# lastz/lastz

Hardware: AMD Instinct MI355X
Metric: Gbp-of-target aligned/sec (whole job, --nogapped HSP path, both strands) (higher is better)
Workload: dtype s32

## Files before the change

lastz_amd/csrc/lz_common.hpp:

```cpp
#pragma once
#include <stdint.h>

#if defined(__HIP__)
#define LZ_HD __host__ __device__ inline __attribute__((always_inline))
#else
#define LZ_HD inline
#endif

typedef uint8_t  u8;
typedef uint32_t u32;
typedef int32_t  s32;
typedef uint64_t u64;
typedef int64_t  s64;

#define LZ_MAX_PARTS   16
#define LZ_MAX_PROBES  128
#define LZ_FILL_GROUP  16
#define LZ_DIAG_BITS   16
#define LZ_DIAG_SIZE   (1u << LZ_DIAG_BITS)
#define LZ_NCLASS      32
#define LZ_SEQ_PAD     64

#define LZ_CODE_CLASS(c)   ((c) & 31u)
#define LZ_CODE_BITS(c)    (((c) >> 5) & 3u)
#define LZ_CODE_INVALID    0x80u

struct LzSeedDev {
    s32 length, weight, nparts;
    s32 shift[LZ_MAX_PARTS];
    u32 mask[LZ_MAX_PARTS];
    s32 nprobes;
    u32 probe_xor[LZ_MAX_PROBES];
};

struct LzHspRec {
    u32 seed_pos1, seed_pos2;
    u32 end1;
    u32 length;
    s32 score;
};

LZ_HD u32 lz_apply_seed(const LzSeedDev& sd, u64 w)
{
    u32 packed = 0;
    for (int p = 0; p < sd.nparts; p++) packed |= (u32)(w >> sd.shift[p]) & sd.mask[p];
    return packed;
}

LZ_HD bool lz_window_word(const u8* code, u32 pos, const LzSeedDev& sd, u32& packed)
{
    u64 w = 0; u32 bad = 0;
    const u8* p = code + pos - (u32)sd.length;
    for (int k = 0; k < sd.length; k++) { u32 c = p[k]; bad |= c; w = (w << 2) | LZ_CODE_BITS(c); }
    if (bad & LZ_CODE_INVALID) return false;
    packed = lz_apply_seed(sd, w);
    return true;
}

LZ_HD u32 lz_count_hits_at(const u8* qcode, u32 pos2, u32 lo, const LzSeedDev& sd, const u32* wstart, bool& valid, u32& packed)
{
    valid = false;
    if (pos2 < lo + (u32)sd.length) return 0;
    if (!lz_window_word(qcode, pos2, sd, packed)) return 0;
    valid = true;
    u32 n = 0;
    for (int p = 0; p < sd.nprobes; p++) { u32 w = packed ^ sd.probe_xor[p]; n += wstart[w + 1] - wstart[w]; }
    return n;
}

LZ_HD u64 lz_hit_key(u32 pos1, u32 pos2) { return ((u64)(u32)(pos1 - pos2) << 32) | (u64)pos2; }

LZ_HD void lz_fill_hits_at(const u8* qcode, u32 pos2, const LzSeedDev& sd, const u32* wstart, const u32* wpos, u64* out)
{
    u32 packed;
    if (!lz_window_word(qcode, pos2, sd, packed)) return;
    for (int p = 0; p < sd.nprobes; p++) {
        u32 w = packed ^ sd.probe_xor[p];
        u32 a = wstart[w], b = wstart[w + 1];
        for (u32 j = a; j < b; j++) *out++ = lz_hit_key(wpos[j], pos2);
    }
}

#define LZ_SELF_OFF       0
#define LZ_SELF_SAME      1
#define LZ_SELF_OPP       2
#define LZ_SELF_OPP_PARTS 3
#define LZ_SELF_WINDOW    4
struct LzSelfDev {
    u32 mode, L, len2, band;
    const u32* sep1; u32 n_sep1;
    u32 wlo;
    const u32* sep2; u32 n_sep2;
// ... 461 lines not shown
```

lastz_amd/csrc/settle_kernels.hip:

```cpp
#include <hip/hip_runtime.h>
#include <cstdio>
#include "lz_ctx.hpp"
#include "lz_lut.hpp"
#include "lz_tile_runs.hpp"
#include "lz_coop.hpp"
#include "lz_seed_dev.hpp"

#define LZ_PP_TPB    1024
#define LZ_PP_WAVES  (LZ_PP_TPB / 64)
#define LZ_PP_ROUNDS (LZ_PP_TILE_HOST / LZ_PP_TPB)
#define LZ_PP_TILE   (LZ_PP_TPB * LZ_PP_ROUNDS)
#define LZ_NBIN      256
static_assert(LZ_PP_TILE == LZ_PP_TILE_HOST, "lz_tile_runs.hpp addresses runs by the tile size");

__device__ __forceinline__ u32 lz_exscan256(u32 v, u32* wtot )
{
    const u32 tid = threadIdx.x, lane = tid & 63u, w = tid >> 6;
    u32 inc = v;
#pragma unroll
    for (int d = 1; d < 64; d <<= 1) { const u32 t = __shfl_up(inc, d); if ((int)lane >= d) inc += t; }
    if (tid < 256 && lane == 63) wtot[w] = inc;
    __syncthreads();
    u32 pre = 0;
    if (tid < 256) for (u32 k = 0; k < w; k++) pre += wtot[k];
// ... 139 lines not shown
                tv = lz_load16(P.tcode + t0); qv = lz_load16(P.qcode + (t0 - diag));
            }
#pragma unroll
            for (int j = 0; j < LZ_COOP_BLK; j++) {
                const u32 tb = right ? LZ_VBYTE(tv, j) : LZ_VBYTE(tv, LZ_COOP_BLK - 1 - j);
                const u32 qb = right ? LZ_VBYTE(qv, j) : LZ_VBYTE(qv, LZ_COOP_BLK - 1 - j);
                sc[j] = tab[(LZ_CODE_CLASS(tb) << 5) | LZ_CODE_CLASS(qb)];
            }
        }
        LzCoopMap f; s32 mx; u32 jmx;
        lz_coop_block(sc, nb, X, f, mx, jmx);
        LzCoopMap inc = f;
#pragma unroll
        for (int d = 1; d < 32; d <<= 1) { const LzCoopMap g = lz_coop_shfl_up32(inc, d); if ((int)hl >= d) inc = lz_coop_compose(g, inc); }
        LzCoopMap ex = lz_coop_shfl_up32(inc, 1);
        if (hl == 0) ex = lz_coop_identity(X);
        const s32 m0 = run0 - best0 + X;
        const bool dead_before = lz_coop_fails(ex, m0);
        const s32 mi = lz_coop_apply(ex, m0), ri = run0 + ex.C;
        const bool fails_here = nb && !dead_before && lz_coop_fails(f, mi);
        const u64 fboth = __ballot(fails_here);
        const u32 fmask = right ? (u32)(fboth >> 32) : (u32)fboth;
        long long key = -1;
        u32 used_here = 0;
        if (fails_here) {
            u32 used; bool stopped; s32 rmx; u32 rj;
            lz_coop_resolve(sc, nb, X, mi, ri, used, stopped, rmx, rj);
            used_here = used;
            if (rj) key = (((long long)rmx + LZ_COOP_INF) << 16) | (long long)(0xFFFFu - (off + rj));
        } else if (nb && jmx && !dead_before)
            key = (((long long)ri + mx + LZ_COOP_INF) << 16) | (long long)(0xFFFFu - (off + jmx));
#pragma unroll
        for (int d = 16; d > 0; d >>= 1) { const long long o = __shfl_xor(key, d, 32); if (o > key) key = o; }
        const int fl = fmask ? (int)__ffs((int)fmask) - 1 : 0;
        const u32 used_f = (u32)__shfl((int)used_here, fl, 32);
        const s32 totc = __shfl(inc.C, 31, 32);
        if (alive) {
            u32 used_total;
            if (fmask) { used_total = LZ_COOP_BLK * (u32)fl + used_f; alive = false; }
            else {
                used_total = room < (u32)(LZ_COOP_BLK * LZ_COOP_LANES) ? room : (u32)(LZ_COOP_BLK * LZ_COOP_LANES);
                if (room <= (u32)(LZ_COOP_BLK * LZ_COOP_LANES)) alive = false;
            }
            if (key >= 0) {
                const s32 v = (s32)((key >> 16) - LZ_COOP_INF); const u32 idx = 0xFFFFu - (u32)(key & 0xFFFF);
                if (v > best0) { best0 = v; out.best_pos = right ? s + idx : s - idx; }
            }
            run0 += totc;
            s = right ? s + used_total : s - used_total;
        }
    }
    out.stop_pos = s; out.best = best0;
    return out;
}

#if defined(LZ_PHASE_CLOCKS)
__device__ unsigned long long g_phase_clk[6];
void lz_phase_clocks_print()
{
    unsigned long long h[6];
    if (hipMemcpyFromSymbol(h, HIP_SYMBOL(g_phase_clk), sizeof(h)) != hipSuccess) return;
    fprintf(stderr, "[lzgpu phase clocks] settle (walker work, walker barrier wait, sorter work, sorter barrier wait, extensions of wave 0: cycles, count; cycles summed over the 256 partitions):");
    for (int k = 0; k < 6; k++) fprintf(stderr, " %llu", h[k]);
    fprintf(stderr, "\n");
}
#define LZ_S2_CLK_BEGIN(who) unsigned long long _s2a = (who) ? __builtin_readcyclecounter() : 0ull, _s2b = 0ull
#define LZ_S2_CLK_MID(who, slot) do { if (who) { _s2b = __builtin_readcyclecounter(); atomicAdd(&g_phase_clk[slot], _s2b - _s2a); } } while (0)
#define LZ_S2_CLK_END(who, slot) do { if (who) atomicAdd(&g_phase_clk[slot], __builtin_readcyclecounter() - _s2b); } while (0)
#define LZ_S2_CLK_EXT_BEGIN(who, m) const unsigned long long _s2x = (who) ? __builtin_readcyclecounter() : 0ull; const unsigned _s2n = (unsigned)__popcll(m)
#define LZ_S2_CLK_EXT_END(who) do { if (who) { atomicAdd(&g_phase_clk[4], __builtin_readcyclecounter() - _s2x); atomicAdd(&g_phase_clk[5], (unsigned long long)_s2n); } } while (0)
#else
#define LZ_S2_CLK_BEGIN(who)
#define LZ_S2_CLK_MID(who, slot)
#define LZ_S2_CLK_END(who, slot)
#define LZ_S2_CLK_EXT_BEGIN(who, m)
#define LZ_S2_CLK_EXT_END(who)
void lz_phase_clocks_print() {}
#endif

#define LZ_S2_TPB     1024
#define LZ_ST_BATCH   4
#define LZ_S2_WALKW   4
#define LZ_S2_SORTW   (LZ_S2_TPB / 64 - LZ_S2_WALKW)
#define LZ_S2_ROUNDS  7
#define LZ_S2_TILE    (LZ_S2_SORTW * 64 * LZ_S2_ROUNDS)
struct LzSettle2Shared {
    s32 tab[LZ_NCLASS * LZ_NCLASS];
    u64 rec[2][LZ_S2_TILE + LZ_ST_BATCH];
    u64 bm[LZ_S2_SORTW][LZ_NBIN];
    u32 cnt[2][LZ_S2_SORTW][LZ_NBIN];
    u32 woff[LZ_S2_SORTW][LZ_NBIN];
    u32 lbeg[2][LZ_NBIN], lcnt[2][LZ_NBIN];
    alignas(8) u8 own[LZ_S2_SORTW][64 * LZ_S2_ROUNDS];
};
static_assert(sizeof(LzSettle2Shared) <= 160 * 1024, "k_settle2: one workgroup per CU");
static_assert(LZ_TR_BLOCK <= 255 && (64 * LZ_S2_ROUNDS) % 8 == 0, "own[] holds 1 + a block entry per byte, cleared 8 at a time");
__global__ void __launch_bounds__(LZ_S2_TPB)
k_settle2(LzExtendParams P, const u64* __restrict__ recs, u32 n_pp_tiles, const u32* __restrict__ hist, const u32* __restrict__ hist_part,
          const u32* __restrict__ run_addr, const u32* __restrict__ bin_base, u32* __restrict__ diag_end,
          const s32* __restrict__ score_tab_g, LzHspRec* __restrict__ out, u32* __restrict__ out_count, u32 out_cap,
          u64* __restrict__ counters)
{
    extern __shared__ __align__(16) unsigned char lz_s2_smem[];
    LzSettle2Shared& sh = *reinterpret_cast<LzSettle2Shared*>(lz_s2_smem);
    const u32 tid = threadIdx.x, lane = tid & 63u;
    const u32 w = (u32)__builtin_amdgcn_readfirstlane((int)(tid >> 6));
    const u32 part = blockIdx.x;
    const u32 r0 = bin_base[part], r1 = bin_base[part + 1];
    const u32 n = r1 - r0, ntiles = (n + LZ_S2_TILE - 1) / LZ_S2_TILE;
    if (ntiles == 0) return;
    for (u32 k = tid; k < LZ_NCLASS * LZ_NCLASS; k += LZ_S2_TPB) sh.tab[k] = score_tab_g[k];
    for (u32 k = tid; k < LZ_S2_SORTW * LZ_NBIN; k += LZ_S2_TPB) (&sh.bm[0][0])[k] = 0ull;
    const bool walker = w < LZ_S2_WALKW;
    const u32 sw = w - LZ_S2_WALKW;

    u64 cx[LZ_S2_ROUNDS], nx[LZ_S2_ROUNDS];
    u32 cslot[LZ_S2_ROUNDS];
    u32 cur = 0, bf[LZ_TR_K], ba[LZ_TR_K];
    auto load_block = [&]() {
#pragma unroll
        for (int j = 0; j < LZ_TR_K; j++) {
            const u32 t = cur + lane * LZ_TR_K + (u32)j;
            bf[j] = lz_tr_first(hist, hist_part, n_pp_tiles, t, part, r1);
            ba[j] = t < n_pp_tiles ? run_addr[(size_t)t * LZ_NBIN + part] : 0u;
        }
    };
    auto block_end = [&]() -> u32 { return (u32)__builtin_amdgcn_readlane((int)bf[LZ_TR_K - 1], 63); };
    auto window_first = [&](u32 tt) -> u32 { return r0 + tt * (u32)LZ_S2_TILE + sw * (64u * LZ_S2_ROUNDS); };
    auto advance_early = [&](u32 tt) {
        if (tt < ntiles && window_first(tt) < r1 && lz_tr_block_behind(block_end(), window_first(tt))) { cur += LZ_TR_BLOCK - 1; load_block(); }
    };
    auto load_tile = [&](u32 tt, u64* x) {
#pragma unroll
        for (int rr = 0; rr < LZ_S2_ROUNDS; rr++) x[rr] = ~0ull;
        const u32 g0 = window_first(tt);
        if (tt >= ntiles || g0 >= r1) return;
        const u32 g1 = (r1 - g0 < 64u * LZ_S2_ROUNDS) ? r1 : g0 + 64u * LZ_S2_ROUNDS;
        u8* const own = sh.own[sw];
        u32 idx[LZ_S2_ROUNDS] = {};
        for (;;) {
            const u32 bend = block_end();
            if (!lz_tr_block_behind(bend, g0)) {
                if (lane < 64u * LZ_S2_ROUNDS / 8u) reinterpret_cast<u64*>(own)[lane] = 0ull;
                u32 dl[LZ_TR_K];
#pragma unroll
                for (int j = 0; j < LZ_TR_K; j++) {
                    const u32 nf = j + 1 < LZ_TR_K ? bf[(j + 1) % LZ_TR_K] : (u32)__shfl_down((int)bf[0], 1);
                    u32 pos;
                    const bool m = lz_tr_mark(bf[j], nf, g0, g1, pos) && !(j == LZ_TR_K - 1 && lane == 63u);
                    if (m) own[pos] = (u8)(1u + lane * LZ_TR_K + (u32)j);
                    dl[j] = lz_tr_delta(ba[j], bf[j]);
                }
                const u32 bfirst = (u32)__builtin_amdgcn_readlane((int)bf[0], 0);
                u32 carry = 0;
#pragma unroll
                for (int rr = 0; rr < LZ_S2_ROUNDS; rr++) {
                    const u32 g = g0 + (u32)rr * 64u + lane;
                    const u32 mk = own[(u32)rr * 64u + lane];
                    u32 v = mk;
                    LZ_WAVE_SCAN_U32(v, mk, lz_umax)
                    v = lz_umax(v, carry);
                    carry = (u32)__builtin_amdgcn_readlane((int)v, 63);
                    const u32 e = v - 1u;
                    u32 d = (u32)__shfl((int)dl[0], (int)(e / LZ_TR_K));
#pragma unroll
                    for (int j = 1; j < LZ_TR_K; j++) { const u32 dj = (u32)__shfl((int)dl[j], (int)(e / LZ_TR_K)); if (e % LZ_TR_K == (u32)j) d = dj; }
                    if (lz_tr_covers(g, bfirst, bend, g1)) idx[rr] = lz_tr_index(g, d);
                }
                if (bend >= g1) break;
            }
            cur += LZ_TR_BLOCK - 1; load_block();
        }
#pragma unroll
        for (int rr = 0; rr < LZ_S2_ROUNDS; rr++)
            if (g0 + (u32)rr * 64u + lane < g1) x[rr] = LZ_NT_LD(recs + (size_t)idx[rr]);
    };
    auto count_tile = [&](u32 tt, const u64* x, u32* slot) {
        u32* const row = sh.cnt[tt & 1u][sw];
        reinterpret_cast<uint4*>(row)[lane] = make_uint4(0u, 0u, 0u, 0u);
        u64* const bmr = sh.bm[sw];
#pragma unroll
        for (int rr = 0; rr < LZ_S2_ROUNDS; rr++) {
            const bool valid = x[rr] != ~0ull;
            const u32 b = LZ_REC_LOW8(x[rr]);
            if (valid) atomicOr((unsigned long long*)&bmr[b], 1ull << lane);
            const u64 peers = valid ? bmr[b] : 0ull;
            const u32 old = valid ? row[b] : 0u;
            const u32 rank = (u32)__popcll(peers & ((1ull << lane) - 1ull));
            if (valid && (peers >> lane) == 1ull) { row[b] = old + (u32)__popcll(peers); bmr[b] = 0ull; }
            slot[rr] = old + rank;
        }
    };
    auto place_tile = [&](u32 tt, const u64* x, const u32* slot) {
        const u32 (*cn)[LZ_NBIN] = sh.cnt[tt & 1u];
        uint4 tot = make_uint4(0u, 0u, 0u, 0u), pre = tot;
#pragma unroll
        for (u32 k = 0; k < LZ_S2_SORTW; k++) {
            const uint4 v = reinterpret_cast<const uint4*>(cn[k])[lane];
            if (k == sw) pre = tot;
            tot.x += v.x; tot.y += v.y; tot.z += v.z; tot.w += v.w;
        }
        const u32 mine = tot.x + tot.y + tot.z + tot.w;
        u32 inc = mine;
#pragma unroll
        for (int d = 1; d < 64; d <<= 1) { const u32 t = __shfl_up(inc, d); if ((int)lane >= d) inc += t; }
        const u32 b0 = inc - mine, b1 = b0 + tot.x, b2 = b1 + tot.y, b3 = b2 + tot.z;
        reinterpret_cast<uint4*>(sh.woff[sw])[lane] = make_uint4(b0 + pre.x, b1 + pre.y, b2 + pre.z, b3 + pre.w);
        if (sw == 0) {
            reinterpret_cast<uint4*>(sh.lbeg[tt & 1u])[lane] = make_uint4(b0, b1, b2, b3);
            reinterpret_cast<uint4*>(sh.lcnt[tt & 1u])[lane] = tot;
        }
        u64* const dst = sh.rec[tt & 1u];
#pragma unroll
        for (int rr = 0; rr < LZ_S2_ROUNDS; rr++)
            if (x[rr] != ~0ull) dst[sh.woff[sw][LZ_REC_LOW8(x[rr])] + slot[rr]] = x[rr];
    };

    __syncthreads();
    if (!walker) {
        load_block();
        load_tile(0, cx); load_tile(1, nx); count_tile(0, cx, cslot);
        __syncthreads();
        place_tile(0, cx, cslot);
#pragma unroll
        for (int rr = 0; rr < LZ_S2_ROUNDS; rr++) cx[rr] = nx[rr];
        load_tile(2, nx);
        count_tile(1, cx, cslot);
        __syncthreads();
        for (u32 t = 0; t < ntiles; t++) {
            LZ_S2_CLK_BEGIN(sw == 0 && lane == 0);
            advance_early(t + 3);
            if (t + 1 < ntiles) place_tile(t + 1, cx, cslot);
#pragma unroll
            for (int rr = 0; rr < LZ_S2_ROUNDS; rr++) cx[rr] = nx[rr];
            load_tile(t + 3, nx);
            if (t + 2 < ntiles) count_tile(t + 2, cx, cslot);
            LZ_S2_CLK_MID(sw == 0 && lane == 0, 2);
            __syncthreads();
            LZ_S2_CLK_END(sw == 0 && lane == 0, 3);
        }
        return;
    }
    __syncthreads();
    __syncthreads();
    constexpr u32 BPW = LZ_NBIN / LZ_S2_WALKW;
    const bool wl = lane < BPW;
    const u32 bucket = (w * BPW + lane) & (LZ_NBIN - 1);
    const u32 h = part * LZ_NBIN + bucket;
    const u32 L = P.seed_len;
    u32 dend = wl ? diag_end[h] : 0u;
    u64 n_ext = 0, n_bp = 0;
    for (u32 t = 0; t < ntiles; t++) {
        LZ_S2_CLK_BEGIN(tid == 0);
        {
            const u64* const rec = sh.rec[t & 1u];
            u32 p = wl ? sh.lbeg[t & 1u][bucket] : 0u; const u32 end = wl ? p + sh.lcnt[t & 1u][bucket] : 0u;
            u32 ne = 0, nb = 0;
            for (;;) {
                bool pending = false; u32 pp2 = 0, ppay = 0;
                while (__ballot(p < end && !pending)) {
                    u64 r[LZ_ST_BATCH];
#pragma unroll
                    for (int k = 0; k < LZ_ST_BATCH; k++) r[k] = rec[p + k];
                    bool live = !pending;
                    u32 np = 0;
#pragma unroll
                    for (int k = 0; k < LZ_ST_BATCH; k++) {
                        const u32 p2 = LZ_REC_POS2(r[k]), pay = LZ_REC_PAYLOAD(r[k]);
                        const bool in = live && (p + (u32)k < end);
                        const bool drop = dend > p2 - L;
                        const bool slow = LZ_REC_SLOW(r[k]) != 0 && !drop;
                        const bool go = in && !slow;
                        const bool fast = go && !drop;
                        const u32 room = p2 - dend, dlo = pay & 0xFFu, dext = pay >> 8;
                        const u32 extent = p2 + dext;
                        ne += fast ? 1u : 0u;
                        nb += fast ? (dlo < room ? dlo : room) + dext : 0u;
                        dend = (fast && extent > dend) ? extent : dend;
                        np += go ? 1u : 0u;
                        if (in && slow) { pending = true; pp2 = p2; ppay = pay; }
                        live = go;
                    }
                    p += np;
                }
                u64 mask = __ballot(pending);
                if (!mask) break;
                LZ_S2_CLK_EXT_BEGIN(tid == 0, mask);
                while (mask) {
                    const int src = (int)__ffsll((long long)mask) - 1;
                    mask &= mask - 1;
                    const u32 sp2 = (u32)__shfl((int)pp2, src), spay = (u32)__shfl((int)ppay, src), sdend = (u32)__shfl((int)dend, src);
                    const u32 sh_ = part * LZ_NBIN + w * BPW + (u32)src;
                    const s32 diag = (s32)((spay << 16) | sh_);
// ... 89 lines not shown
```

lastz_amd/csrc/lz_lut.hpp:

```cpp
#pragma once
#include "lz_common.hpp"

#define LZ_PAD2         128
#define LZ_LUT_ENTRIES  4096
#define LZ_LUT_TOTAL    (2 * LZ_LUT_ENTRIES)
#define LZ_LUT_WIN_G    15
#define LZ_LUT_WIN_B    60
#define LZ_LUT_MAXWIN   3
#define LZ_GRAY(c)      ((c) ^ ((c) >> 1))

struct alignas(8) LzLutEntry { u32 ab; u32 sc; };

struct LzLutParams {
    const u8* t2; const u8* q2;
    const u8* tsp; const u8* qsp;
    const u8* t2x; const u8* tspx;
    const u8* tcode; const u8* qcode;
    s32 xdrop;
};

struct LzLutScan { u32 s; s32 run, best; u32 room, used, alive, nwin; };

#if defined(__HIP_DEVICE_COMPILE__)
LZ_HD u32 lz_alignbit(u32 hi, u32 lo, u32 sh) { return __builtin_amdgcn_alignbit(hi, lo, sh); }
// ... 123 lines not shown
            stop = stop | (on && nr < best - X);
        }
    } else if (r) {
        const s32 p1 = lz_sdot4m(sc, 0x00000001u, m), p2 = lz_sdot4m(sc, 0x00000101u, m), p3 = lz_sdot4m(sc, 0x00010101u, m), p4 = lz_sdot4(sc, m);
        const s32 q2 = p1 | p2, q3 = q2 | p3;
        j = 4u + (u32)(p1 >> 31) + (u32)(q2 >> 31) + (u32)(q3 >> 31);
        stop = (q3 | p4) < 0;
    }
    st.run = run; st.best = best;
    st.used += 4u * np + j;
    st.nwin++;
    if (stop) st.alive = 0;
    else if (r == 4u) st.alive = 2;
    else if (soft) {
        if constexpr (SPECIAL) {
            const u32 p1 = RIGHT ? st.s + lim : st.s - 1u - lim;
            const s32 v = ctab[(LZ_CODE_CLASS(P.tcode[(s64)p1]) << 5) | LZ_CODE_CLASS(P.qcode[(s64)p1 - (s64)diag])];
            st.run += v; st.used += 1u;
            if (st.run > st.best) st.best = st.run;
            const u32 eaten = lim + 1u;
            if (st.run < st.best - X || eaten == st.room) st.alive = 0;
            else { st.alive = 1; st.room -= eaten; st.s = RIGHT ? st.s + eaten : st.s - eaten; }
        }
    }
    else if (lim == st.room) st.alive = 0;
    else { st.alive = 1; st.room -= (u32)LZ_LUT_WIN_B; st.s = RIGHT ? st.s + (u32)LZ_LUT_WIN_B : st.s - (u32)LZ_LUT_WIN_B; }
}
template <bool SPECIAL, bool LIMCHK>
LZ_HD void lz_lut_window_pair(const LzLutParams& P, const LzLutEntry* lut, s32 diag, LzLutScan& L, LzLutScan& R,
                              const LzLutRaw<SPECIAL>& rawl, const LzLutRaw<SPECIAL>& rawr, bool do_l, bool do_r, const s32* ctab = nullptr)
{
    if (do_l) lz_lut_window<false, SPECIAL, LIMCHK>(P, lut, diag, L, rawl, ctab);
    if (do_r) lz_lut_window<true, SPECIAL, LIMCHK>(P, lut, diag, R, rawr, ctab);
}
template <bool RIGHT, bool SPECIAL>
LZ_HD void lz_lut_step(const LzLutParams& P, const LzLutEntry* lut, s32 diag, LzLutScan& st, const s32* ctab = nullptr)
{
    LzLutRaw<SPECIAL> raw;
    lz_lut_fetch<RIGHT, SPECIAL>(P, st.s, diag, raw);
    if (!SPECIAL && st.room >= (u32)LZ_LUT_WIN_B) lz_lut_window<RIGHT, SPECIAL, false>(P, lut, diag, st, raw);
    else                                           lz_lut_window<RIGHT, SPECIAL, true>(P, lut, diag, st, raw, ctab);
}

LZ_HD void lz_lut_init(u64 key, u32 tlen, u32 qlen, s32& diag, LzLutScan& L, LzLutScan& R)
{
    const u32 pos2 = (u32)key;
    diag = (s32)(u32)(key >> 32);
    const u32 pos1 = pos2 + (u32)diag;
    const s32 stopl = diag > 0 ? diag : 0;
    const s32 stopr = ((s32)tlen <= (s32)qlen + diag) ? (s32)tlen : (s32)qlen + diag;
    L.s = R.s = pos1; L.run = L.best = R.run = R.best = 0; L.used = R.used = 0; L.nwin = R.nwin = 0;
    L.room = (u32)((s32)pos1 - stopl); R.room = (u32)(stopr - (s32)pos1);
    L.alive = ((s32)pos1 > stopl) ? 1u : 0u; R.alive = ((s32)pos1 < stopr) ? 1u : 0u;
}

LZ_HD u32 lz_lut_summary(const LzLutScan& L, const LzLutScan& R, s32 min_score)
{
    u32 summ = (L.used & 0xFFu) | ((R.used & 0xFFu) << 8);
    if (L.alive || R.alive || L.best + R.best >= min_score) summ |= LZ_SUMM_SLOW;
    return summ;
}

template <bool SPECIAL>
LZ_HD u32 lz_lut_probe_hit(const LzLutParams& P, const LzLutEntry* lut, u32 tlen, u32 qlen, s32 min_score, u64 key, const s32* ctab = nullptr)
{
    s32 diag; LzLutScan L, R;
    lz_lut_init(key, tlen, qlen, diag, L, R);
    while (L.alive == 1 && L.nwin < (u32)LZ_LUT_MAXWIN) lz_lut_step<false, SPECIAL>(P, lut, diag, L, ctab);
    while (R.alive == 1 && R.nwin < (u32)LZ_LUT_MAXWIN) lz_lut_step<true, SPECIAL>(P, lut, diag, R, ctab);
    return lz_lut_summary(L, R, min_score);
}

LZ_HD u64 lz_hit_record(u64 key, u32 summ)
{
    const u32 pos2 = (u32)key, diag = (u32)(key >> 32);
    const bool slow = (summ & LZ_SUMM_SLOW) != 0;
    const u64 payload = slow ? (u64)(diag >> 16) : (u64)(summ & 0xFFFFu);
    return (u64)pos2 | ((u64)(diag & 0xFFu) << 31) | (payload << 39) | (slow ? (1ull << 63) : 0ull);
}
#define LZ_REC_TAG(r)     ((u32)((r) >> 55) & 0xFFu)
#define LZ_REC_UNTAG(r)   ((r) & ~(0xFFull << 55))
LZ_HD u64 lz_hit_record_tagged(u64 key, u32 summ) { return lz_hit_record(key, summ) | ((u64)((u32)(key >> 40) & 0xFFu) << 55); }

#define LZ_WCTX_BYTES 32
struct alignas(16) LzWctx { u32 w[LZ_WCTX_BYTES / 4]; };
LZ_HD u32 lz_wctx_first_byte(u32 pos1) { return ((pos1 - 1u + (u32)LZ_PAD2) >> 2) - 15u; }
LZ_HD u32 lz_wctx_right_offset(u32 pos1) { return ((pos1 + (u32)LZ_PAD2) >> 2) - lz_wctx_first_byte(pos1); }
LZ_HD LzWctx lz_wctx_make(const u8* two, u32 pos1) { LzWctx e; __builtin_memcpy(&e, two + lz_wctx_first_byte(pos1), LZ_WCTX_BYTES); return e; }
LZ_HD void lz_wctx_windows(const LzWctx& e, u32 pos1, LzVec16& tl, LzVec16& tr)
{
    const bool at16 = lz_wctx_right_offset(pos1) == 16u;
    LZ_UNROLL_ALL
    for (int k = 0; k < 4; k++) {
        tl.w[k] = e.w[k];
        const u32 at15 = lz_alignbit(e.w[4 + k], e.w[3 + k], 24u);
        tr.w[k] = at16 ? e.w[4 + k] : at15;
    }
}

#define LZ_REC_POS2(r)    ((u32)((r) & 0x7FFFFFFFu))
#define LZ_REC_LOW8(r)    ((u32)((r) >> 31) & 0xFFu)
#define LZ_REC_PAYLOAD(r) ((u32)((r) >> 39) & 0xFFFFu)
#define LZ_REC_SLOW(r)    ((u32)((r) >> 63))
LZ_HD u64 lz_rec_with_index(u64 r, u32 idx)
{ return (r & ~((0xFFull << 31) | (0x1Full << 55))) | ((u64)(idx & 0xFFu) << 31) | ((u64)((idx >> 8) & 0x1Fu) << 55); }
#define LZ_REC_INDEX(r)   (((u32)((r) >> 31) & 0xFFu) | (((u32)((r) >> 55) & 0x1Fu) << 8))

template <class Emit>
LZ_HD void lz_settle_record(const LzExtendParams& P, const s32* score_tab, u64 rec, u32 h ,
                            u32& dend, u64& n_ext, u64& n_bp, Emit&& emit)
{
    const u32 p2 = LZ_REC_POS2(rec);
    if (dend > p2 - P.seed_len) return;
    n_ext++;
    const u32 pay = LZ_REC_PAYLOAD(rec);
    if (!LZ_REC_SLOW(rec)) {
        const u32 room = p2 - dend, dlo = pay & 0xFFu, dext = pay >> 8;
        const u32 extent = p2 + dext;
        n_bp += (dlo < room ? dlo : room) + dext;
        if (extent > dend) dend = extent;
        return;
    }
    const s32 diag = (s32)((pay << 16) | h);
    dend = lz_reextend(P, score_tab, p2, diag, dend, n_bp, emit);
}
```

lastz_amd/csrc/scan_kernels.hip:

```cpp
#include <hip/hip_runtime.h>
#include <algorithm>
#include <type_traits>
#include "lz_ctx.hpp"
#include "lz_host.hpp"
#include "lz_lut.hpp"
#include "lz_seed_dev.hpp"

#define LZ_SC_ROUNDS 4

struct LzScanTask { u32 idx; s32 diag; LzLutScan L, R; };
static_assert(sizeof(LzScanTask) == 64, "LzScanTask: one 64-byte line per task");
#define LZ_SC_TPB 512
template <int MODE> struct LzScanShared {
    union {
        LzLutEntry lut[LZ_LUT_TOTAL];
        struct { s32 tab[LZ_NCLASS * LZ_NCLASS]; s32 tab8[64]; } bc;
    };
    s32 ctab[MODE == 1 ? LZ_NCLASS * LZ_NCLASS : 1];
};

template <bool SP>
__device__ __forceinline__ void lz_scan_round(const LzExtendParams& P, const LzLutParams& Q, const LzLutEntry* lut, const s32* ctab, u64 key, bool valid,
                                              const LzLutRaw<SP>& rawl, const LzLutRaw<SP>& rawr, u32 idx, u32 lane,
                                              u32& summ_out, LzScanTask* __restrict__ my_tasks, u32& my_n, u32 region_cap)
{
    constexpr bool HLIM = SP;
    s32 diag; LzLutScan L, R;
    lz_lut_init(key, P.tlen, P.qlen, diag, L, R);
    if (!valid) { L.alive = 0; R.alive = 0; }
    const bool ql = L.alive && !HLIM && L.room < (u32)LZ_LUT_WIN_B, qr = R.alive && !HLIM && R.room < (u32)LZ_LUT_WIN_B;
    lz_lut_window_pair<SP, HLIM>(Q, lut, diag, L, R, rawl, rawr, L.alive && !ql, R.alive && !qr, ctab);
    const bool more = valid && (L.alive == 1 || R.alive == 1);
    const u64 mm = __ballot(more);
    bool queued = false;
    if (mm) {
        const u32 slot = my_n + (u32)__popcll(mm & ((1ull << lane) - 1ull));
        if (more && slot < region_cap) {
            LzScanTask t; t.idx = idx; t.diag = diag; t.L = L; t.R = R;
            my_tasks[slot] = t; queued = true;
        }
        my_n += (u32)__popcll(mm);
    }
    summ_out = queued ? 0u : lz_lut_summary(L, R, P.min_score);
}
template <bool SP>
__device__ __forceinline__ void lz_scan_fetch(const LzLutParams& Q, u64 key, LzLutRaw<SP>& rawl, LzLutRaw<SP>& rawr)
{
    const u32 pos2 = (u32)key, pos1 = pos2 + (u32)(key >> 32);
    const s32 diag = (s32)(u32)(key >> 32);
    const u32 stl = pos1 - 1u + (u32)LZ_PAD2, str = pos1 + (u32)LZ_PAD2;
    const u32 bl = (stl >> 2) - 15u, br = str >> 2;
    const u32 ol = bl + (bl & ~31u);
    rawl.tv = lz_load16(Q.t2x + ol); rawr.tv = lz_load16(Q.t2x + (ol + (br - bl)));
    const u32 sql = stl - (u32)diag, sqr = str - (u32)diag;
    rawl.qv = lz_load16(Q.q2 + ((sql >> 2) - 15u)); rawr.qv = lz_load16(Q.q2 + (sqr >> 2));
    if constexpr (SP) {
        const u32 ml = (stl >> 3) - 14u, mr = str >> 3;
        const u32 oml = ml + (ml & ~31u);
        rawl.tm = lz_load16(Q.tspx + oml); rawr.tm = lz_load16(Q.tspx + (oml + (mr - ml)));
        rawl.qm = lz_load16(Q.qsp + ((sql >> 3) - 14u)); rawr.qm = lz_load16(Q.qsp + (sqr >> 3));
    }
}

template <int MODE, int TPB, int WPE>
__global__ void __launch_bounds__(TPB, WPE)
k_scan_hits(LzExtendParams P, LzLutParams Q, const u64* __restrict__ keys, u64 n,
            const s32* __restrict__ score_tab_g, const LzLutEntry* __restrict__ lut_g,
            u32* __restrict__ summ, u8* __restrict__ bins, LzScanTask* __restrict__ tasks, u32* __restrict__ n_tasks, u32 region_cap)
{
    __shared__ LzScanShared<MODE> sh;
    const u32 tid = threadIdx.x, lane = tid & 63u, w = tid >> 6;
    if (MODE == 1) { for (u32 k = tid; k < LZ_NCLASS * LZ_NCLASS; k += TPB) sh.ctab[k] = score_tab_g[k]; }
    if (MODE < 2) { for (u32 k = tid; k < LZ_LUT_TOTAL; k += TPB) sh.lut[k] = lut_g[k]; }
    else {
        for (u32 k = tid; k < LZ_NCLASS * LZ_NCLASS; k += TPB) sh.bc.tab[k] = score_tab_g[k];
        if (tid < 64) sh.bc.tab8[tid] = score_tab_g[(tid >> 3) * LZ_NCLASS + (tid & 7)];
    }
    __syncthreads();
    const LzLutEntry* lut = sh.lut;
    const s32* const ctab = sh.ctab;
    constexpr bool SP = MODE == 1;
    constexpr u32 SPAN = 64u * LZ_SC_ROUNDS;
    static_assert(LZ_SC_ROUNDS == 4, "the round pipeline below is written out for four rounds per span");
    const u64 nspans = (n + SPAN - 1) / SPAN, wstride = (u64)gridDim.x * (TPB / 64);
    const u32 region = blockIdx.x * (TPB / 64) + w;
    LzScanTask* const my_tasks = tasks + (size_t)region * region_cap;
    u32 my_n = 0;
    u64 span = (u64)blockIdx.x * (TPB / 64) + w;
    if (MODE == 2) {
        for (; span < nspans; span += wstride) {
            const u64 base = span * SPAN;
            const u32 span_n = (n - base < (u64)SPAN) ? (u32)(n - base) : SPAN;
#pragma unroll 1
            for (u32 r = 0; r < LZ_SC_ROUNDS; r++) {
                const u32 li = r * 64u + lane;
                if (li < span_n) { const u64 kk = keys[base + li]; summ[base + li] = lz_probe_hit(P, sh.bc.tab, sh.bc.tab8, P.cls8 != 0, kk); bins[base + li] = (u8)LZ_KEY_BIN(kk); }
            }
        }
    } else if (span < nspans) {
        typedef u64 lz_u64x2 __attribute__((ext_vector_type(2)));
        auto load_keys = [&](u64 sp, u64& a0, u64& a1, u64& a2, u64& a3) {
            const u64 base = sp * SPAN;
            const u32 sn = (n - base < (u64)SPAN) ? (u32)(n - base) : SPAN;
            const u32 l4 = 4u * lane;
            const u64* kp = keys + base + l4;
            if (l4 + 3u < sn) {
                const lz_u64x2 x = LZ_NT_LD(reinterpret_cast<const lz_u64x2*>(kp)), y = LZ_NT_LD(reinterpret_cast<const lz_u64x2*>(kp + 2));
                a0 = x.x; a1 = x.y; a2 = y.x; a3 = y.y;
            } else {
                a0 = (l4 < sn) ? LZ_NT_LD(kp) : 0ull;           a1 = (l4 + 1u < sn) ? LZ_NT_LD(kp + 1) : 0ull;
                a2 = (l4 + 2u < sn) ? LZ_NT_LD(kp + 2) : 0ull;  a3 = 0ull;
            }
        };
        u64 k0, k1, k2, k3;
        load_keys(span, k0, k1, k2, k3);
        LzLutRaw<SP> al, ar, bl, br;
        lz_scan_fetch<SP>(Q, k0, al, ar);
#pragma unroll 1
        for (;;) {
            const u64 base = span * SPAN;
            const u32 span_n = (n - base < (u64)SPAN) ? (u32)(n - base) : SPAN;
            const u32 l4 = 4u * lane;
            const u32 ib = (u32)base + l4;
            const bool more_spans = span + wstride < nspans;
            u64 n0 = 0, n1 = 0, n2 = 0, n3 = 0;
            u32 s0, s1, s2, s3;
            lz_scan_fetch<SP>(Q, k1, bl, br);
            lz_scan_round<SP>(P, Q, lut, ctab, k0, l4 < span_n, al, ar, ib, lane, s0, my_tasks, my_n, region_cap);
            if (more_spans) load_keys(span + wstride, n0, n1, n2, n3);
            lz_scan_fetch<SP>(Q, k2, al, ar);
            lz_scan_round<SP>(P, Q, lut, ctab, k1, l4 + 1u < span_n, bl, br, ib + 1u, lane, s1, my_tasks, my_n, region_cap);
            lz_scan_fetch<SP>(Q, k3, bl, br);
            lz_scan_round<SP>(P, Q, lut, ctab, k2, l4 + 2u < span_n, al, ar, ib + 2u, lane, s2, my_tasks, my_n, region_cap);
            if (more_spans) lz_scan_fetch<SP>(Q, n0, al, ar);
            lz_scan_round<SP>(P, Q, lut, ctab, k3, l4 + 3u < span_n, bl, br, ib + 3u, lane, s3, my_tasks, my_n, region_cap);
            const u32 pbytes = LZ_KEY_BIN(k0) | (LZ_KEY_BIN(k1) << 8) | (LZ_KEY_BIN(k2) << 16) | (LZ_KEY_BIN(k3) << 24);
            if (l4 + 3u < span_n) {
                typedef u32 lz_u32x4 __attribute__((ext_vector_type(4)));
                lz_u32x4 sv4; sv4.x = s0; sv4.y = s1; sv4.z = s2; sv4.w = s3;
                LZ_NT_ST(sv4, reinterpret_cast<lz_u32x4*>(summ + ib));
                LZ_NT_ST(pbytes, reinterpret_cast<u32*>(bins + ib));
            } else {
                if (l4 < span_n)      { summ[ib] = s0;      bins[ib] = (u8)pbytes; }
                if (l4 + 1u < span_n) { summ[ib + 1u] = s1; bins[ib + 1u] = (u8)(pbytes >> 8); }
                if (l4 + 2u < span_n) { summ[ib + 2u] = s2; bins[ib + 2u] = (u8)(pbytes >> 16); }
            }
            if (!more_spans) break;
            span += wstride; k0 = n0; k1 = n1; k2 = n2; k3 = n3;
        }
    }
    if (lane == 0) n_tasks[region] = my_n < region_cap ? my_n : region_cap;
}

#define LZ_ST_TPB 512
template <int MODE, bool TAGGED>
__global__ void __launch_bounds__(LZ_ST_TPB)
k_scan_tasks(LzExtendParams P, LzLutParams Q, const LzLutEntry* __restrict__ lut_g, const s32* __restrict__ score_tab_g, const LzScanTask* __restrict__ tasks,
             const u32* __restrict__ n_tasks, u32 n_regions, u32 region_cap, std::conditional_t<TAGGED, u64, u32>* __restrict__ out)
{
    constexpr bool SP = MODE == 1;
    static_assert(!(SP && TAGGED), "pos1 is recovered from the windows a scan ran: without special bytes only");
    __shared__ LzLutEntry lut[LZ_LUT_TOTAL];
    __shared__ s32 ctab[SP ? LZ_NCLASS * LZ_NCLASS : 1];
    for (u32 k = threadIdx.x; k < LZ_LUT_TOTAL; k += LZ_ST_TPB) lut[k] = lut_g[k];
    if (SP) for (u32 k = threadIdx.x; k < LZ_NCLASS * LZ_NCLASS; k += LZ_ST_TPB) ctab[k] = score_tab_g[k];
    __syncthreads();
    for (u32 region = blockIdx.x; region < n_regions; region += gridDim.x) {
        const u32 nt = n_tasks[region];
        for (u32 k = threadIdx.x; k < nt; k += (u32)LZ_ST_TPB) {
            const LzScanTask t = tasks[(size_t)region * region_cap + k];
            LzLutScan L = t.L, R = t.R;
            u32 pos1 = 0;
            if constexpr (TAGGED) pos1 = L.alive == 1 ? L.s + (u32)LZ_LUT_WIN_B * L.nwin : R.s - (u32)LZ_LUT_WIN_B * R.nwin;
            while (L.alive == 1 && L.nwin < (u32)LZ_LUT_MAXWIN) lz_lut_step<false, SP>(Q, lut, t.diag, L, ctab);
            while (R.alive == 1 && R.nwin < (u32)LZ_LUT_MAXWIN) lz_lut_step<true, SP>(Q, lut, t.diag, R, ctab);
            const u32 summ = lz_lut_summary(L, R, P.min_score);
            if constexpr (TAGGED) out[t.idx] = lz_hit_record_tagged(lz_hit_key(pos1, pos1 - (u32)t.diag), summ);
            else                  LZ_NT_ST(summ, out + t.idx);
        }
    }
}

static int lz_scan_tpb(int mode)
{
    return mode != 0 ? LZ_SC_TPB : 640;
}
static int lz_task_regions(LzCtx& c, int mode, u64 n, u32 n_regions, u32& region_cap)
{
    region_cap = (u32)std::min<u64>(n / (mode == 1 ? 12 : 32) / n_regions + 64, 1u << 20);
    if (const u32 force = lz_settings().task_region_cap) region_cap = force;
    int rc;
    if (mode < 2 && (rc = c.scan_tasks.ensure((size_t)n_regions * region_cap * sizeof(LzScanTask)))) return rc;
    return c.scan_ntasks.ensure((size_t)n_regions * 4);
}
static int lz_scan_buffers(LzCtx& c, int mode, u64 n, u32& grid, u32& n_regions, u32& region_cap)
{
    const u32 wpg = (u32)lz_scan_tpb(mode) / 64u;
    const int cus = c.num_cus;
    const u64 nspans = (n + 64u * LZ_SC_ROUNDS - 1) / (64u * LZ_SC_ROUNDS), want = (nspans + wpg - 1) / wpg;
    grid = (u32)std::min<u64>(want ? want : 1, 2u * (u64)cus);
    n_regions = grid * wpg;
    const int rc = c.summ.ensure((size_t)n * 4);
    return rc ? rc : lz_task_regions(c, mode, n, n_regions, region_cap);
}
int lzk_scan_reserve(LzCtx& c, int mode, u64 max_n)
{
    u32 grid, n_regions, region_cap;
    return lz_scan_buffers(c, mode, max_n, grid, n_regions, region_cap);
}

int lzk_scan_hits(LzCtx& c, int mode, const LzExtendParams& P, const LzLutParams& Q, u64 n)
{
    if (n == 0) return 0;
    const int cus = c.num_cus;
    int rc;
    u32 grid, n_regions, task_cap;
    if ((rc = lz_scan_buffers(c, mode, n, grid, n_regions, task_cap))) return rc;
    const u64* keys = c.keys.as<u64>(); const s32* score_tab = c.score_tab.as<s32>(); const LzLutEntry* lut = c.lut.as<LzLutEntry>();
    u32* summ = c.summ.as<u32>(); u8* bins = c.bins.as<u8>(); LzScanTask* tasks = c.scan_tasks.as<LzScanTask>(); u32* ntk = c.scan_ntasks.as<u32>();
    c.timer.begin("k_scan_hits", c.stream);
#define LZ_SCAN_LAUNCH(M_, T_, W_) hipLaunchKernelGGL((k_scan_hits<M_, T_, W_>), dim3(grid), dim3(T_), 0, c.stream, P, Q, keys, n, score_tab, lut, summ, bins, tasks, ntk, task_cap)
    if (mode == 0)      LZ_SCAN_LAUNCH(0, 640, 5);
    else if (mode == 1) LZ_SCAN_LAUNCH(1, LZ_SC_TPB, 4);
    else                LZ_SCAN_LAUNCH(2, LZ_SC_TPB, 4);
#undef LZ_SCAN_LAUNCH
    c.timer.end(c.stream);
    LZ_HIP(hipGetLastError());
    if (mode < 2) {
        const dim3 tgrid(std::min<u32>(n_regions, 4u * (u32)cus));
        c.timer.begin("k_scan_tasks", c.stream);
        if (mode == 0) hipLaunchKernelGGL((k_scan_tasks<0, false>), tgrid, dim3(LZ_ST_TPB), 0, c.stream, P, Q, lut, score_tab, tasks, ntk, n_regions, task_cap, summ);
        else           hipLaunchKernelGGL((k_scan_tasks<1, false>), tgrid, dim3(LZ_ST_TPB), 0, c.stream, P, Q, lut, score_tab, tasks, ntk, n_regions, task_cap, summ);
        c.timer.end(c.stream);
        LZ_HIP(hipGetLastError());
    }
    return 0;
}

struct LzFuseTrip { u32 p1, pos2, dst; bool ok; LzWctx cx; LzVec16 ql, qr; };

template <bool SELF, int TPB, int CAP>
__global__ void __launch_bounds__(TPB)
k_scan_hits2(u32 lo, u32 i0, u32 i1, LzSeedDev sd,
             const u32* __restrict__ wstart, const u32* __restrict__ wpos, const LzWctx* __restrict__ wctx,
             const u32* __restrict__ sk, const u32* __restrict__ sv, u32 n, const u64* __restrict__ off, u64 base,
             LzExtendParams P, LzLutParams Q, const LzLutEntry* __restrict__ lut_g,
             u64* __restrict__ recs, LzScanTask* __restrict__ tasks, u32* __restrict__ n_tasks, u32 region_cap, LzSelfDev self)
{
    __shared__ LzLutEntry lut[LZ_LUT_TOTAL];
    constexpr int WORDS = CAP / 2 / 64;
    __shared__ LzListWave<CAP> shw[TPB / 64];
    for (u32 k = threadIdx.x; k < LZ_LUT_TOTAL; k += TPB) lut[k] = lut_g[k];
    __syncthreads();
    LzListWave<CAP>& sh = shw[threadIdx.x >> 6];
    unsigned short* const own = reinterpret_cast<unsigned short*>(sh.own32);
    const u32 lane = threadIdx.x & 63u;
    const u32 region = blockIdx.x * (TPB / 64) + (threadIdx.x >> 6), nwaves = gridDim.x * (TPB / 64);
    LzScanTask* const my_tasks = tasks + (size_t)region * region_cap;
    u32 my_n = 0;
    const u32 ngroups = (n + 63u) / 64u;
    for (u32 grp = region; grp < ngroups; grp += nwaves) {
        const u32 j = grp * 64u + lane;
        u32 w_l = 0, i_l = 0; bool in = false;
        if (j < n) { w_l = sk[j] & ((2u << sd.weight) - 1u); i_l = sv[j]; in = !(w_l >> sd.weight) && i_l >= i0 && i_l < i1; }
        if (!__ballot(in)) continue;
        const u32 dbase = in ? (u32)(off[i_l] - base) : 0u;
        const u32 pos2 = lo + i_l + 1u;
        u32 slo = 0, shi = 0;
        if (SELF) lz_self_bounds(self, pos2, slo, shi);
        u32 carry = 0;
        for (int r = 0; r < sd.nprobes; r += LZ_FILL_GROUP) {
#include "lz_enum_place.inc"
            for (u32 cs = 0; cs < T; cs += CAP) {
                const u32 tc = (T - cs < (u32)CAP) ? T - cs : (u32)CAP;
#include "lz_enum_owners.inc"
                auto load_trip = [&](u32 tb, LzFuseTrip& t) {
                    const u32 t0 = tb + lane;
                    t.ok = t0 < tc;
                    const u32 tt = t.ok ? t0 : tc - 1u;
                    const u32 list = (u32)own[tt] - 1u;
                    const u32 ls = sh.lsrc[list];
                    const uint2 en = sh.ent[list / LZ_FILL_GROUP];
                    const u32 tabs = cs + tt, e = ls + tabs;
                    t.p1 = wpos[e]; t.cx = wctx[e];
                    t.pos2 = en.y; t.dst = en.x + tabs;
                    const u32 sql = en.y - 1u + (u32)LZ_PAD2;
                    t.ql = lz_load16(Q.q2 + ((sql >> 2) - 15u)); t.qr = lz_load16(Q.q2 + ((sql + 1u) >> 2));
                };
                auto scan_trip = [&](const LzFuseTrip& t) {
                    const u64 key = lz_hit_key(t.p1, t.pos2);
                    LzLutRaw<false> rl, rr;
                    lz_wctx_windows(t.cx, t.p1, rl.tv, rr.tv);
                    rl.qv = t.ql; rr.qv = t.qr;
                    u32 summ;
                    lz_scan_round<false>(P, Q, lut, nullptr, key, t.ok, rl, rr, t.dst, lane, summ, my_tasks, my_n, region_cap);
                    if (t.ok) LZ_NT_ST(lz_hit_record_tagged(key, summ), recs + t.dst);
                };
                LzFuseTrip ta, tb2;
                load_trip(0u, ta);
#pragma unroll 1
                for (u32 tb = 0;;) {
                    if (tb + 64u < tc) load_trip(tb + 64u, tb2);
                    scan_trip(ta);
                    tb += 64u; if (tb >= tc) break;
                    if (tb + 64u < tc) load_trip(tb + 64u, ta);
                    scan_trip(tb2);
                    tb += 64u; if (tb >= tc) break;
                }
                __atomic_signal_fence(__ATOMIC_SEQ_CST);
            }
            carry += total;
        }
    }
    if (lane == 0) n_tasks[region] = my_n < region_cap ? my_n : region_cap;
}

static u32 lz_fused_tpb(LzCtx& c)
{
    return c.self.mode != LZ_SELF_OFF ? 512u : 1024u;
}
static int lz_fused_buffers(LzCtx& c, u64 n_hits, u32& grid, u32& n_regions, u32& region_cap)
{
    const int cus = c.num_cus;
    grid = (u32)cus; n_regions = grid * (lz_fused_tpb(c) / 64u);
    return lz_task_regions(c, 0, n_hits, n_regions, region_cap);
}
int lzk_fused_reserve(LzCtx& c, u64 max_n)
{
    u32 grid, n_regions, region_cap;
    return lz_fused_buffers(c, max_n, grid, n_regions, region_cap);
}
int lzk_scan_fused(LzCtx& c, u32 lo, const LzChunk& ch, u32 n, const LzExtendParams& P, const LzLutParams& Q)
{
    if (n == 0 || ch.i1 <= ch.i0 || ch.nh == 0) return 0;
    const u32* sk = c.wsk.as<u32>(); const u32* sv = c.wsv.as<u32>();
    lz_chunk_range(c, ch.i0, ch.i1, sk, sv, n);
    if (n == 0) return 0;
    int rc;
    u32 grid, n_regions, region_cap;
    if ((rc = lz_fused_buffers(c, ch.nh, grid, n_regions, region_cap))) return rc;
    const LzLutEntry* lut = c.lut.as<LzLutEntry>(); u64* tagged = c.keys.as<u64>();
    LzScanTask* tasks = c.scan_tasks.as<LzScanTask>(); u32* ntk = c.scan_ntasks.as<u32>();
    c.timer.begin("k_scan_hits", c.stream);
#define LZ_FUSED_LAUNCH(S_, T_, C_, self_) hipLaunchKernelGGL((k_scan_hits2<S_, T_, C_>), dim3(grid), dim3(T_), 0, c.stream, lo, ch.i0, ch.i1, c.seed, c.wstart.as<u32>(), c.wpos.as<u32>(), \
                           c.wctx.as<LzWctx>(), sk, sv, n, c.off.as<u64>(), ch.base, P, Q, lut, tagged, tasks, ntk, region_cap, self_)
    if (c.self.mode != LZ_SELF_OFF) LZ_FUSED_LAUNCH(true, 512, 2560, c.self);
    else                            LZ_FUSED_LAUNCH(false, 1024, 512, LzSelfDev{});
#undef LZ_FUSED_LAUNCH
    c.timer.end(c.stream);
    LZ_HIP(hipGetLastError());
    c.timer.begin("k_scan_tasks", c.stream);
    hipLaunchKernelGGL((k_scan_tasks<0, true>), dim3(std::min<u32>(n_regions, 4u * grid)), dim3(LZ_ST_TPB), 0, c.stream, P, Q, lut, (const s32*)nullptr, tasks, ntk, n_regions, region_cap, tagged);
    c.timer.end(c.stream);
    LZ_HIP(hipGetLastError());
    return 0;
}
```

Measured before the change: 0.4073.

## Shrink settle2 LDS bookkeeping to 16 bits and enlarge the sort tile

After: 0.4050. About the same (-0.6%).

```diff
diff --git a/lastz_amd/csrc/lz_common.hpp b/lastz_amd/csrc/lz_common.hpp
--- a/lastz_amd/csrc/lz_common.hpp
+++ b/lastz_amd/csrc/lz_common.hpp
@@ -8,6 +8,7 @@
 #endif
 
 typedef uint8_t  u8;
+typedef uint16_t u16;
 typedef uint32_t u32;
 typedef int32_t  s32;
 typedef uint64_t u64;
diff --git a/lastz_amd/csrc/settle_kernels.hip b/lastz_amd/csrc/settle_kernels.hip
--- a/lastz_amd/csrc/settle_kernels.hip
+++ b/lastz_amd/csrc/settle_kernels.hip
@@ -245,19 +245,23 @@
 #define LZ_ST_BATCH   4
 #define LZ_S2_WALKW   4
 #define LZ_S2_SORTW   (LZ_S2_TPB / 64 - LZ_S2_WALKW)
-#define LZ_S2_ROUNDS  7
+#ifndef LZ_S2_ROUNDS
+#define LZ_S2_ROUNDS  9
+#endif
 #define LZ_S2_TILE    (LZ_S2_SORTW * 64 * LZ_S2_ROUNDS)
+typedef uint2 __attribute__((may_alias)) lz_u16x4;
 struct LzSettle2Shared {
     s32 tab[LZ_NCLASS * LZ_NCLASS];
     u64 rec[2][LZ_S2_TILE + LZ_ST_BATCH];
     u64 bm[LZ_S2_SORTW][LZ_NBIN];
-    u32 cnt[2][LZ_S2_SORTW][LZ_NBIN];
-    u32 woff[LZ_S2_SORTW][LZ_NBIN];
-    u32 lbeg[2][LZ_NBIN], lcnt[2][LZ_NBIN];
-    alignas(8) u8 own[LZ_S2_SORTW][64 * LZ_S2_ROUNDS];
+    u16 cnt[2][LZ_S2_SORTW][LZ_NBIN];
+    u16 woff[LZ_S2_SORTW][LZ_NBIN];
+    u16 lbeg[2][LZ_NBIN], lcnt[2][LZ_NBIN];
 };
 static_assert(sizeof(LzSettle2Shared) <= 160 * 1024, "k_settle2: one workgroup per CU");
-static_assert(LZ_TR_BLOCK <= 255 && (64 * LZ_S2_ROUNDS) % 8 == 0, "own[] holds 1 + a block entry per byte, cleared 8 at a time");
+static_assert(LZ_S2_TILE + LZ_ST_BATCH < 65536, "cnt, woff, lbeg, lcnt: counts and offsets inside one tile, in 16 bits");
+static_assert(LZ_TR_BLOCK <= 255 && (64 * LZ_S2_ROUNDS) % 16 == 0 && 64 * LZ_S2_ROUNDS / 16 <= 64 && 64 * LZ_S2_ROUNDS <= LZ_NBIN * 8,
+              "own[] holds 1 + a block entry per byte, cleared 16 per lane by one wave, inside a row of bm");
 __global__ void __launch_bounds__(LZ_S2_TPB)
 k_settle2(LzExtendParams P, const u64* __restrict__ recs, u32 n_pp_tiles, const u32* __restrict__ hist, const u32* __restrict__ hist_part,
           const u32* __restrict__ run_addr, const u32* __restrict__ bin_base, u32* __restrict__ diag_end,
@@ -299,12 +303,11 @@
         const u32 g0 = window_first(tt);
         if (tt >= ntiles || g0 >= r1) return;
         const u32 g1 = (r1 - g0 < 64u * LZ_S2_ROUNDS) ? r1 : g0 + 64u * LZ_S2_ROUNDS;
-        u8* const own = sh.own[sw];
+        u8* const own = reinterpret_cast<u8*>(sh.bm[sw]);
         u32 idx[LZ_S2_ROUNDS] = {};
         for (;;) {
             const u32 bend = block_end();
             if (!lz_tr_block_behind(bend, g0)) {
-                if (lane < 64u * LZ_S2_ROUNDS / 8u) reinterpret_cast<u64*>(own)[lane] = 0ull;
                 u32 dl[LZ_TR_K];
 #pragma unroll
                 for (int j = 0; j < LZ_TR_K; j++) {
@@ -330,6 +333,9 @@
                     for (int j = 1; j < LZ_TR_K; j++) { const u32 dj = (u32)__shfl((int)dl[j], (int)(e / LZ_TR_K)); if (e % LZ_TR_K == (u32)j) d = dj; }
                     if (lz_tr_covers(g, bfirst, bend, g1)) idx[rr] = lz_tr_index(g, d);
                 }
+                if (lane < 64u * LZ_S2_ROUNDS / 16u) {
+                    reinterpret_cast<u64*>(own)[2u * lane] = 0ull; reinterpret_cast<u64*>(own)[2u * lane + 1u] = 0ull;
+                }
                 if (bend >= g1) break;
             }
             cur += LZ_TR_BLOCK - 1; load_block();
@@ -339,8 +345,8 @@
             if (g0 + (u32)rr * 64u + lane < g1) x[rr] = LZ_NT_LD(recs + (size_t)idx[rr]);
     };
     auto count_tile = [&](u32 tt, const u64* x, u32* slot) {
-        u32* const row = sh.cnt[tt & 1u][sw];
-        reinterpret_cast<uint4*>(row)[lane] = make_uint4(0u, 0u, 0u, 0u);
+        u16* const row = sh.cnt[tt & 1u][sw];
+        reinterpret_cast<lz_u16x4*>(row)[lane] = make_uint2(0u, 0u);
         u64* const bmr = sh.bm[sw];
 #pragma unroll
         for (int rr = 0; rr < LZ_S2_ROUNDS; rr++) {
@@ -350,28 +356,29 @@
             const u64 peers = valid ? bmr[b] : 0ull;
             const u32 old = valid ? row[b] : 0u;
             const u32 rank = (u32)__popcll(peers & ((1ull << lane) - 1ull));
-            if (valid && (peers >> lane) == 1ull) { row[b] = old + (u32)__popcll(peers); bmr[b] = 0ull; }
+            if (valid && (peers >> lane) == 1ull) { row[b] = (u16)(old + (u32)__popcll(peers)); bmr[b] = 0ull; }
             slot[rr] = old + rank;
         }
     };
     auto place_tile = [&](u32 tt, const u64* x, const u32* slot) {
-        const u32 (*cn)[LZ_NBIN] = sh.cnt[tt & 1u];
+        const u16 (*cn)[LZ_NBIN] = sh.cnt[tt & 1u];
         uint4 tot = make_uint4(0u, 0u, 0u, 0u), pre = tot;
 #pragma unroll
         for (u32 k = 0; k < LZ_S2_SORTW; k++) {
-            const uint4 v = reinterpret_cast<const uint4*>(cn[k])[lane];
+            const uint2 v = reinterpret_cast<const lz_u16x4*>(cn[k])[lane];
             if (k == sw) pre = tot;
-            tot.x += v.x; tot.y += v.y; tot.z += v.z; tot.w += v.w;
+            tot.x += v.x & 0xFFFFu; tot.y += v.x >> 16; tot.z += v.y & 0xFFFFu; tot.w += v.y >> 16;
         }
         const u32 mine = tot.x + tot.y + tot.z + tot.w;
         u32 inc = mine;
 #pragma unroll
         for (int d = 1; d < 64; d <<= 1) { const u32 t = __shfl_up(inc, d); if ((int)lane >= d) inc += t; }
         const u32 b0 = inc - mine, b1 = b0 + tot.x, b2 = b1 + tot.y, b3 = b2 + tot.z;
-        reinterpret_cast<uint4*>(sh.woff[sw])[lane] = make_uint4(b0 + pre.x, b1 + pre.y, b2 + pre.z, b3 + pre.w);
+        auto pack4 = [](u32 a, u32 b, u32 c, u32 d) -> uint2 { return make_uint2(a | (b << 16), c | (d << 16)); };
+        reinterpret_cast<lz_u16x4*>(sh.woff[sw])[lane] = pack4(b0 + pre.x, b1 + pre.y, b2 + pre.z, b3 + pre.w);
         if (sw == 0) {
-            reinterpret_cast<uint4*>(sh.lbeg[tt & 1u])[lane] = make_uint4(b0, b1, b2, b3);
-            reinterpret_cast<uint4*>(sh.lcnt[tt & 1u])[lane] = tot;
+            reinterpret_cast<lz_u16x4*>(sh.lbeg[tt & 1u])[lane] = pack4(b0, b1, b2, b3);
+            reinterpret_cast<lz_u16x4*>(sh.lcnt[tt & 1u])[lane] = pack4(tot.x, tot.y, tot.z, tot.w);
         }
         u64* const dst = sh.rec[tt & 1u];
 #pragma unroll
```

## Drain queued scan tasks inside fused kernel in full 64-lane batches

Applied to the files above, without the earlier changes.

Measured after the change: 0.4078 before, 0.4146 after (median of 6 runs). 1.7% higher.

```diff
diff --git a/lastz_amd/csrc/lz_lut.hpp b/lastz_amd/csrc/lz_lut.hpp
--- a/lastz_amd/csrc/lz_lut.hpp
+++ b/lastz_amd/csrc/lz_lut.hpp
@@ -229,6 +229,22 @@
 #define LZ_REC_UNTAG(r)   ((r) & ~(0xFFull << 55))
 LZ_HD u64 lz_hit_record_tagged(u64 key, u32 summ) { return lz_hit_record(key, summ) | ((u64)((u32)(key >> 40) & 0xFFu) << 55); }
 
+struct LzScanTask { u32 idx; s32 diag; LzLutScan L, R; };
+static_assert(sizeof(LzScanTask) == 64, "LzScanTask: one 64-byte line per task");
+template <bool SPECIAL, bool TAGGED>
+LZ_HD u64 lz_lut_task(const LzLutParams& P, const LzLutEntry* lut, const s32* ctab, const LzScanTask& t, s32 min_score)
+{
+    static_assert(!(SPECIAL && TAGGED), "pos1 is recovered from the windows a scan ran: without special bytes only");
+    LzLutScan L = t.L, R = t.R;
+    u32 pos1 = 0;
+    if constexpr (TAGGED) pos1 = L.alive == 1 ? L.s + (u32)LZ_LUT_WIN_B * L.nwin : R.s - (u32)LZ_LUT_WIN_B * R.nwin;
+    while (L.alive == 1 && L.nwin < (u32)LZ_LUT_MAXWIN) lz_lut_step<false, SPECIAL>(P, lut, t.diag, L, ctab);
+    while (R.alive == 1 && R.nwin < (u32)LZ_LUT_MAXWIN) lz_lut_step<true, SPECIAL>(P, lut, t.diag, R, ctab);
+    const u32 summ = lz_lut_summary(L, R, min_score);
+    if constexpr (TAGGED) return lz_hit_record_tagged(lz_hit_key(pos1, pos1 - (u32)t.diag), summ);
+    else                  return (u64)summ;
+}
+
 #define LZ_WCTX_BYTES 32
 struct alignas(16) LzWctx { u32 w[LZ_WCTX_BYTES / 4]; };
 LZ_HD u32 lz_wctx_first_byte(u32 pos1) { return ((pos1 - 1u + (u32)LZ_PAD2) >> 2) - 15u; }
diff --git a/lastz_amd/csrc/scan_kernels.hip b/lastz_amd/csrc/scan_kernels.hip
--- a/lastz_amd/csrc/scan_kernels.hip
+++ b/lastz_amd/csrc/scan_kernels.hip
@@ -8,8 +8,6 @@
 
 #define LZ_SC_ROUNDS 4
 
-struct LzScanTask { u32 idx; s32 diag; LzLutScan L, R; };
-static_assert(sizeof(LzScanTask) == 64, "LzScanTask: one 64-byte line per task");
 #define LZ_SC_TPB 512
 template <int MODE> struct LzScanShared {
     union {
@@ -19,10 +17,10 @@
     s32 ctab[MODE == 1 ? LZ_NCLASS * LZ_NCLASS : 1];
 };
 
-template <bool SP>
+template <bool SP, bool QOUT = false>
 __device__ __forceinline__ void lz_scan_round(const LzExtendParams& P, const LzLutParams& Q, const LzLutEntry* lut, const s32* ctab, u64 key, bool valid,
                                               const LzLutRaw<SP>& rawl, const LzLutRaw<SP>& rawr, u32 idx, u32 lane,
-                                              u32& summ_out, LzScanTask* __restrict__ my_tasks, u32& my_n, u32 region_cap)
+                                              u32& summ_out, LzScanTask* __restrict__ my_tasks, u32& my_n, u32 region_cap, bool* queued_out = nullptr)
 {
     constexpr bool HLIM = SP;
     s32 diag; LzLutScan L, R;
@@ -42,6 +40,7 @@
         my_n += (u32)__popcll(mm);
     }
     summ_out = queued ? 0u : lz_lut_summary(L, R, P.min_score);
+    if constexpr (QOUT) *queued_out = queued;
 }
 template <bool SP>
 __device__ __forceinline__ void lz_scan_fetch(const LzLutParams& Q, u64 key, LzLutRaw<SP>& rawl, LzLutRaw<SP>& rawr)
@@ -167,7 +166,8 @@
     __syncthreads();
     for (u32 region = blockIdx.x; region < n_regions; region += gridDim.x) {
         const u32 nt = n_tasks[region];
-        for (u32 k = threadIdx.x; k < nt; k += (u32)LZ_ST_TPB) {
+        const u32 k0 = TAGGED ? nt & ~63u : 0u;
+        for (u32 k = k0 + threadIdx.x; k < nt; k += (u32)LZ_ST_TPB) {
             const LzScanTask t = tasks[(size_t)region * region_cap + k];
             LzLutScan L = t.L, R = t.R;
             u32 pos1 = 0;
@@ -238,6 +238,11 @@
 }
 
 struct LzFuseTrip { u32 p1, pos2, dst; bool ok; LzWctx cx; LzVec16 ql, qr; };
+__device__ __forceinline__ void lz_scan_task_tagged(const LzLutParams& Q, const LzLutEntry* lut, const LzScanTask* __restrict__ tp, s32 min_score, u64* __restrict__ recs)
+{
+    const LzScanTask t = *tp;
+    recs[t.idx] = lz_lut_task<false, true>(Q, lut, nullptr, t, min_score);
+}
 
 template <bool SELF, int TPB, int CAP>
 __global__ void __launch_bounds__(TPB)
@@ -257,7 +262,13 @@
     const u32 lane = threadIdx.x & 63u;
     const u32 region = blockIdx.x * (TPB / 64) + (threadIdx.x >> 6), nwaves = gridDim.x * (TPB / 64);
     LzScanTask* const my_tasks = tasks + (size_t)region * region_cap;
-    u32 my_n = 0;
+    u32 my_n = 0, done = 0;
+    auto drain = [&]() {
+        __builtin_amdgcn_fence(__ATOMIC_RELEASE, "workgroup");
+        __builtin_amdgcn_fence(__ATOMIC_ACQUIRE, "workgroup");
+        lz_scan_task_tagged(Q, lut, my_tasks + (done + lane), P.min_score, recs);
+        done += 64u;
+    };
     const u32 ngroups = (n + 63u) / 64u;
     for (u32 grp = region; grp < ngroups; grp += nwaves) {
         const u32 j = grp * 64u + lane;
@@ -292,9 +303,9 @@
                     LzLutRaw<false> rl, rr;
                     lz_wctx_windows(t.cx, t.p1, rl.tv, rr.tv);
                     rl.qv = t.ql; rr.qv = t.qr;
-                    u32 summ;
-                    lz_scan_round<false>(P, Q, lut, nullptr, key, t.ok, rl, rr, t.dst, lane, summ, my_tasks, my_n, region_cap);
-                    if (t.ok) LZ_NT_ST(lz_hit_record_tagged(key, summ), recs + t.dst);
+                    u32 summ; bool queued;
+                    lz_scan_round<false, true>(P, Q, lut, nullptr, key, t.ok, rl, rr, t.dst, lane, summ, my_tasks, my_n, region_cap, &queued);
+                    if (t.ok && !queued) LZ_NT_ST(lz_hit_record_tagged(key, summ), recs + t.dst);
                 };
                 LzFuseTrip ta, tb2;
                 load_trip(0u, ta);
@@ -311,6 +322,7 @@
             }
             carry += total;
         }
+        while ((my_n < region_cap ? my_n : region_cap) - done >= 64u) drain();
     }
     if (lane == 0) n_tasks[region] = my_n < region_cap ? my_n : region_cap;
 }
```
